# lan496/torch-m3gnet

Measured on AMD Instinct MI355X. Metric: atom-steps/sec (energy+forces) on 10k-atom PBC batch, 1/2/4/8 MI355X, higher is better.
Workload: dtype f32; 1 GPU; single 10000-atom fcc Cu PBC supercell per GPU (10x10x25 cells, a=3.61 A, jitter 0.025 A), r_cut 5 A / 3-body 4 A, default M3GNet (l_max=n_max=3, D=64, 3 blocks), energy+forces+stress; precision=fp32, atoms_per_gpu=10000, edges_per_gpu=420000, triplets_per_gpu=3060000

## Files before the change

torch-m3gnet_amd/csrc/m3g_api.hip:

```cpp
#include <climits>
#include <cmath>
#include <cstdarg>
#include <cstdio>
#include <cstdlib>
#include <cstring>
#include <utility>

#include "m3g_internal.h"

namespace m3g {

static thread_local char g_err[512] = "";
void set_error(const char* fmt, ...) {
  va_list ap;
  va_start(ap, fmt);
  vsnprintf(g_err, sizeof(g_err), fmt, ap);
  va_end(ap);
}

static void layout_mlp(MlpW& m, size_t& off) {
  auto take = [&](size_t n) { size_t r = off; off += (n + 63) / 64 * 64; return r; };
  m.w1a_t = take(kDP * 2 * kDP); m.w1b_t = take(kDP * 2 * kDP); m.w1c_t = take(kDP * 2 * kDP);
  m.b1 = take(2 * kDP);
  m.w2d_t = take(kDP * kDP); m.w2g_t = take(kDP * kDP);
// ... 304 lines not shown
  *value = *value == 0 ? 0 : *value == 3 ? 3 : *value == 2 ? 2 : 1;
  return M3G_OK;
}
struct OptionRow {
  const char* name;
  int Options::*member;
  int lo, hi;
  const char* error;
  int (*hook)(m3g_plan*, int32_t* value);
};
#define M3G_HOOK(...) [](m3g_plan* plan, int32_t* value) -> int { __VA_ARGS__; return M3G_OK; }
static const OptionRow kOptions[] = {
    {"edge_kernel", &Options::edge_kernel, 0, 2, "edge_kernel must be 0 (VALU baseline), 1 (MFMA) or 2 (any-size path)",
     M3G_HOOK(if (plan->generic && *value != 2) { set_error("this model size only runs on the any-size path (edge_kernel = 2)"); return M3G_ERR_UNSUPPORTED; })},
    {"precision", &Options::precision, 0, 2,
     "precision must be 0 (fp32: exact fp32 MFMA products), 1 (bf16x3 split products) or 2 (f16x3: scaled fp16 split products)", nullptr},
    {"save_p1", &Options::save_p1, 0, 1, nullptr, nullptr},
    {"save_p2", &Options::save_p2, 0, 1, nullptr, nullptr},
    {"rev_kernel", &Options::rev_kernel, 0, 1, "rev_kernel must be 0 (node-MLP + edge-MLP kernel pair) or 1 (fused)", nullptr},
    {"small_tiles", &Options::small_tiles, 0, INT_MAX, "small_tiles must be >= 0", M3G_HOOK(plan->opt.small_tiles_fwd = *value)},
    {"small_tiles_fwd", &Options::small_tiles_fwd, 0, INT_MAX, "small_tiles_fwd must be >= 0", nullptr},
    {"dp1_by_dst", &Options::dp1_by_dst, 0, 1, nullptr, nullptr},
    {"split_node_tiles", &Options::split_node_tiles, 0, INT_MAX, "split_node_tiles must be >= 0", nullptr},
    {"fuse_node_tb", &Options::fuse_node_tb, 0, 1, nullptr, nullptr},
    {"debug_node_tb_polls", &Options::debug_node_tb_polls, INT_MIN, INT_MAX, nullptr, nullptr},
    {"split_tail", &Options::split_tail, 0, 2, "split_tail must be 0 (never), 1 (a single left-over tile) or 2 (one or two)", nullptr},
    {"small_launches", &Options::small_launches, 0, 1, nullptr, nullptr},
    {"graph_replay", &Options::graph_replay, 0, 1, nullptr, M3G_HOOK(if (!*value) drop_graphs(plan))},
    {"overlap", &Options::overlap, 0, 1, nullptr, nullptr},
    {"threebody_moments", &Options::tb_moments, 0, 1, nullptr, nullptr},
    {"legendre_backward", &Options::legendre_ref, 0, 1, "legendre_backward: 0 (exact derivative) or 1 (the reference's backward)", nullptr},
    {"readout_f16", &Options::readout_f16, 0, 1, nullptr, nullptr},
    {"stress_mode", &Options::stress_mode, 0, 1, "stress_mode must be 0 (reference: sum pos (x) F / V) or 1 (pair virial)", nullptr},
    {"debug_force_move", nullptr, INT_MIN, INT_MAX, nullptr, M3G_HOOK(plan->debug_force_move = *value != 0; plan->committed = false)},
    {"stamps", &Options::stamp_target, INT_MIN, INT_MAX, nullptr, hook_stamps},
};
#undef M3G_HOOK

extern "C" int m3g_plan_set_option(m3g_plan* plan, const char* name, int32_t value) {
  if (!plan || !name) { set_error("m3g_plan_set_option: null argument"); return M3G_ERR_VALUE; }
  for (const OptionRow& row : kOptions) {
    if (strcmp(name, row.name) != 0) continue;
    if (value < row.lo || value > row.hi) {
      if (row.error) { set_error("%s", row.error); return M3G_ERR_VALUE; }
      value = 1;
    }
// ... 81 lines not shown
    std::string ro = buf;
    const float* wd0 = plan->params.at(ro + ".dense.0.weight").data();
    const float* wg0 = plan->params.at(ro + ".gate.0.weight").data();
    const float* wd2 = plan->params.at(ro + ".dense.2.weight").data();
    const float* wg2 = plan->params.at(ro + ".gate.2.weight").data();
    put_t(blob, r.w1d_t, kDP, wd0, D, D, 0, D); put_t(blob, r.w1g_t, kDP, wg0, D, D, 0, D);
    put_t(blob, r.w2d_t, kDP, wd2, D, D, 0, D); put_t(blob, r.w2g_t, kDP, wg2, D, D, 0, D);
    put_n(blob, r.w1d, kDP, wd0, D, D, 0, D); put_n(blob, r.w1g, kDP, wg0, D, D, 0, D);
    put_n(blob, r.w2d, kDP, wd2, D, D, 0, D); put_n(blob, r.w2g, kDP, wg2, D, D, 0, D);
    for (int o = 0; o < D; ++o) {
      blob[r.b1d + o] = plan->params.at(ro + ".dense.0.bias")[o];
      blob[r.b1g + o] = plan->params.at(ro + ".gate.0.bias")[o];
      blob[r.b2d + o] = plan->params.at(ro + ".dense.2.bias")[o];
      blob[r.b2g + o] = plan->params.at(ro + ".gate.2.bias")[o];
      blob[r.w3d + o] = plan->params.at(ro + ".dense.4.weight")[o];
      blob[r.w3g + o] = plan->params.at(ro + ".gate.4.weight")[o];
    }
    blob[r.b3] = plan->params.at(ro + ".dense.4.bias")[0];
    blob[r.b3 + 1] = plan->params.at(ro + ".gate.4.bias")[0];
  }
  if (!plan->d_weights) M3G_HIP_CHECK(hipMalloc((void**)&plan->d_weights, wl.total * sizeof(float)));
  M3G_HIP_CHECK(hipMemcpy(plan->d_weights, blob.data(), wl.total * sizeof(float), hipMemcpyHostToDevice));
  { int rc = pack_mfma_images(plan); if (rc) return rc; }
  plan->committed = true;
  return M3G_OK;
}

static StepPath plan_step_path(const m3g_plan* plan, int64_t N, int64_t E, int64_t T, int64_t S, int topo_hints, bool forces, bool stresses, bool profile) {
  const m3g_config& cfg = plan->cfg;
  return resolve_step_path(plan->opt, ModelDims{cfg.l_max, cfg.n_max, cfg.l_max * cfg.n_max, cfg.num_blocks}, N, E, T, S, topo_hints, forces, stresses, profile);
}

extern "C" int m3g_workspace_bytes(const m3g_plan* plan, int64_t N, int64_t E, int64_t T, int64_t S, size_t* bytes) {
  if (!plan || !bytes || N < 0 || E < 0 || T < 0 || S < 0) { set_error("m3g_workspace_bytes: bad argument"); return M3G_ERR_VALUE; }
  const StepPath p = plan_step_path(plan, N, E, T, S, 0, true, true, false);
  *bytes = p.pipeline == kPipeAnySize ? generic_workspace_bytes(plan, N, E, T, S) : work_carve(plan->cfg.num_blocks, p, N, E, S, nullptr).total_bytes;
  return M3G_OK;
}

static bool ensure_side_stream(const m3g_plan* plan) {
  if (plan->side_stream) return true;
  if (hipStreamCreateWithFlags(&plan->side_stream, hipStreamNonBlocking) != hipSuccess) { plan->side_stream = nullptr; return false; }
  if (hipEventCreateWithFlags(&plan->ev_fork, hipEventDisableTiming) != hipSuccess ||
      hipEventCreateWithFlags(&plan->ev_join, hipEventDisableTiming) != hipSuccess)
    return false;
  return true;
// ... 19 lines not shown
  const float* W;
  hipStream_t s;
  RunMode mode;
  Topo t;
  Work w;
  float *ea, *st;
  int enqueue_forward() const, enqueue_optional_outputs() const, enqueue_reverse() const;
};

static int check_call(const m3g_plan* plan, const m3g_io* io) {
  if (!plan || !io) { set_error("m3g_energy_forces: null argument"); return M3G_ERR_VALUE; }
  if (!plan->committed) { set_error("m3g_energy_forces: plan parameters not committed"); return M3G_ERR_STATE; }
  int dev = -1;
  M3G_HIP_CHECK(hipGetDevice(&dev));
  if (dev == plan->device) return M3G_OK;
  set_error("m3g_energy_forces: the plan was committed on device %d but the current device is %d (commit again on this device)", plan->device, dev);
  return M3G_ERR_STATE;
}

int Step::enqueue_forward() const {
  const bool want_f = io->forces != nullptr;
  {
    M3G_STAGE(ST_GEOM);
    if (p.geom_with_node_pre) launch_geometry_node_pre(plan, c, t, w, io->pos, io->lattice, io->edge_cell_shift, io->atom_types, W + wl.emb, s);
    else launch_geometry(c, t, io->pos, io->lattice, io->edge_cell_shift, w, s);
  }
  {
    M3G_STAGE(ST_EMBED);
    if (mfma) {
      if (c.B == 0) launch_embed_nodes_only(c, W, wl, t, io->atom_types, w, s);
      if (!p.fused_rev || c.B == 0) launch_embed_edges_soa(c, W + wl.adj_t, w.h, w.e_blk[0], t.E, s);
    } else {
      launch_embed(c, W, wl, t, io->atom_types, w, s);
    }
  }
  for (int b = 0; b < c.B; ++b) {
    {
      M3G_STAGE(ST_NODE_PRE);
      if (mfma && b == 0 && p.geom_with_node_pre) {  }
      else if (mfma) launch_node_pre_mfma(plan, p.node_split, c, t, w, b, b > 0 ? w.x[b - 1] : nullptr, w.x[b], w.v[b], w.TAb[b], w.TBb[b],
                                          b == 0 ? io->atom_types : nullptr, W + wl.emb, s);
      else launch_node_pre(c, W, wl.blk[b], t, w, nullptr, w.x[b], w.v[b], w.TA, w.TB, s);
    }
    { M3G_STAGE(ST_THREEBODY); launch_threebody(p, c, t, w, w.v[b], w.m[b], s); }
    M3G_STAGE(ST_EDGE_FWD);
    if (mfma) {
      if (p.fwd_split) launch_edge_fwd_split(plan, p, c, t, w, b, s);
      else launch_edge_block_mfma(plan, p, c, t, w, b, s);
      (void)ST_NODE_SUM;
    } else {
      launch_edge_block(c, W, wl.blk[b], t, w, b, w.x[b], w.x[b + 1], s);
    }
  }
  M3G_STAGE(ST_READOUT);
  if (mfma) launch_readout_mfma(plan, p, c, wl, t, io->atom_types, c.B > 0 ? w.x[c.B - 1] : nullptr, w.x[c.B], w, ea, st, io->total_energy, want_f, s);
  else launch_readout(c, W, wl, t, io->atom_types, nullptr, w.x[c.B], w, ea, st, io->total_energy, want_f, s);
  return M3G_OK;
}

int Step::enqueue_optional_outputs() const {
  M3G_STAGE(ST_OUTPUTS);
  if (io->node_features) launch_copy_strided(w.x[c.B], kDP, io->node_features, c.D, c.D, t.N, s);
  if (io->edge_attr) {
    if (mfma) launch_soa_to_rows(w.e_blk[c.B], io->edge_attr, c.D, c.D, t.E, s);
    else launch_copy_strided(w.e, kDP, io->edge_attr, c.D, c.D, t.E, s);
  }
  if (io->edge_distances && t.E > 0) M3G_HIP_CHECK(hipMemcpyAsync(io->edge_distances, w.d, sizeof(float) * t.E, hipMemcpyDeviceToDevice, s));
  if (io->edge_weights) launch_copy_strided(w.h, kRP, io->edge_weights, c.R, c.R, t.E, s);
  if (io->triplet_angles) launch_triplet_angles(t, io->triplet_edge_index, w.u, io->triplet_angles, s);
  if (io->mid_edge_features)
    for (int b = 0; b < c.B; ++b)
// ... 215 lines not shown
```

torch-m3gnet_amd/csrc/m3g_edge_mfma.hip:

```cpp
#include "m3g_edge_common.h"

namespace m3g {

__device__ __forceinline__ void save_store(float* ptr, const f32x4& val) { __builtin_nontemporal_store(val, (f32x4*)ptr); }
template <bool KEEP_P1, int PREC, int SAVE = 0>
__device__ __forceinline__ void mlp_preacts(const float* lds, int w1c, int w2d, int w2g, int b2, const f32x4 (&x)[4], f32x4 (&p1)[8],
                                            f32x4 (&p2)[8], int lane, float* p1_out = nullptr, float* p2_out = nullptr, float w_inv = 1.f) {
  chain_p<PREC, 8, 2>(lds + w1c, x, p1, lane, w_inv);
  if constexpr (SAVE == 1) static_for<8>([&]<int ob>() { *(f32x4*)(p1_out + ob * 256) = p1[ob]; });
  bias_step<4, 0>(lds + b2, p2, lane);
  bias_step<4, 4>(lds + b2 + 4 * 64, p2, lane);
  if constexpr (!KEEP_P1 && SAVE == 2) {
    static_for<8>([&]<int ob>() {
      f32x4 ds;
      static_for<2>([&]<int k>() {
        f32x2 act, der;
        silu_pair(f32x2{p1[ob][2 * k], p1[ob][2 * k + 1]}, act, der);
        p1[ob][2 * k] = act[0]; p1[ob][2 * k + 1] = act[1];
        ds[2 * k] = der[0]; ds[2 * k + 1] = der[1];
      });
      save_store(p1_out + ob * 256, ds);
    });
    chain_p<PREC, 4, 2, 0, 0>(lds + w2d, p1, p2, lane, w_inv);
    chain_p<PREC, 4, 2, 4, 4>(lds + w2g, p1, p2, lane, w_inv);
// ... 17 lines not shown
      static_for<8>([&]<int ob>() { static_for<4>([&]<int r>() { p1[ob][r] = fsilu(p1[ob][r]); }); });
    }
    chain_p<PREC, 4, 2, 0, 0>(lds + w2d, p1, p2, lane, w_inv);
    chain_p<PREC, 4, 2, 4, 4>(lds + w2g, p1, p2, lane, w_inv);
  }
}

template <bool ST, int S0, int PREC, int SAVE>
__device__ __forceinline__ void mlp_forward_mfma(const float* lds, const MfmaMlpFwd& L, int mlp, const FwdArgs& a, int64_t ci,
                                                 int64_t cj, float hb, const f32x4 (&x)[4], f32x4 (&out)[4], int lane,
                                                 Stamps<ST>& st, float* p1_out, float* p2_out) {
  f32x4 p1[8], p2[8];
  gather_tables(a.TA, a.TB, mlp, ci, cj, lane >> 4, p1);
  st.template mark<S0>();
  mlp_preacts<false, PREC, SAVE>(lds, L.w1c, L.w2d, L.w2g, L.b2, x, p1, p2, lane, p1_out, p2_out, a.w_inv);
  st.template mark<S0 + 1>();
  static_for<4>([&]<int ob>() {
    out[ob] = mfma16(lds[L.wl + ob * 64 + lane], hb, zero4());
    mul_gated<PREC == kPrecF16x3 || PREC == kPrecF32>(out[ob], p2[ob], p2[4 + ob]);
  });
  st.template mark<S0 + 3>();
}

template <int TBS, bool ST = false, bool FIRST = false, int PREC = kPrecBf16x3, int SAVE = 0>
__global__ void __launch_bounds__(64 * fwd_waves<PREC>()) k_edge_block_mfma(FwdArgs a, MfmaFwdLayout L) {
  __shared__ __attribute__((aligned(16))) float lds[kFwdLdsFloats + 4];
  int* q_head = reinterpret_cast<int*>(lds + kFwdLdsFloats);
  load_image(lds, a.img, kFwdLdsFloats, q_head);
  const int lane = threadIdx.x & 63, qd = lane >> 4;
  TileQueue queue(a.tiles, q_head);
  Stamps<ST> st;
  int ticket = queue.fetch(lane);
  if (ticket >= queue.count) return;
  int ci_i, cj_i;
  load_ends(a.src, a.dst, queue.base + ticket, a.E, lane, ci_i, cj_i);
  int arow_i = load_arow(a.act_id, queue.base + ticket, a.E, lane);
  for (;;) {
    const int64_t tile = queue.base + ticket;
    ticket = queue.fetch(lane);
    const bool has_next = ticket < queue.count;
    int nci = 0, ncj = 0, narow = -1;
    if (has_next) {
      load_ends(a.src, a.dst, queue.base + ticket, a.E, lane, nci, ncj);
      narow = load_arow(a.act_id, queue.base + ticket, a.E, lane);
    }
    int lv = lane;
    asm volatile("" : "+v"(lv));
// ... 9 lines not shown
    if (!FIRST) static_for<4>([&]<int blk>() { x[blk] = load_tile4(e_tile + blk * 256); });
    const int arow = arow_i;
    const TbIn<PREC, TBS> tbin = tb_load<PREC, TBS>(a.m, arow, qv, a.w_inv);
    const float hb = a.h[ec * kRP + qv];
    if (FIRST) {
      static_for<4>([&]<int blk>() {
        x[blk] = mfma16(lds[L.adj + blk * 64 + lv], hb, zero4());
        static_for<4>([&]<int r>() { x[blk][r] = fsilu(x[blk][r]); });
      });
    }
    st.template mark<0>();
    {
      f32x4 p[8];
      tb_preact_p<PREC, TBS>(lds + L.tb, tbin, p, lv);
      static_for<4>([&]<int blk>() { add_gated<PREC == kPrecF16x3 || PREC == kPrecF32>(x[blk], p[blk], p[4 + blk]); });
    }
    st.template mark<1>();
    f32x4 out[4];
    float* p1_tile = SAVE >= 1 ? a.p1_out + tile * (2 * kP1TileFloats) + lane * 4 : nullptr;
    float* p2_tile = SAVE >= 2 ? a.p2_out + tile * (2 * kP1TileFloats) + lane * 4 : nullptr;
    mlp_forward_mfma<ST, 2, PREC, SAVE>(lds, L.mlp[0], 0, a, ci, cj, hb, x, out, lv, st, p1_tile, p2_tile);
    static_for<4>([&]<int blk>() {
      x[blk] += out[blk];
      *(f32x4*)(e_otile + blk * 256) = x[blk];
    });
    st.template mark<6>();
    mlp_forward_mfma<ST, 7, PREC, SAVE>(lds, L.mlp[1], 1, a, ci, cj, hb, x, out, lv, st, SAVE >= 1 ? p1_tile + kP1TileFloats : nullptr,
                                        SAVE >= 2 ? p2_tile + kP1TileFloats : nullptr);
    {
      if (edge >= a.E) static_for<4>([&]<int blk>() { out[blk] = zero4(); });
      const SegMasks sk = seg_masks((int)ci, lane);
      seg_scan(out, sk);
      seg_store(out, sk, a.seg_head, a.seg_first, tile, ci, qd, 0);
    }
    st.template mark<11>();
    if (!has_next) break;
    ci_i = nci;
    cj_i = ncj;
    arow_i = narow;
  }
  st.template store<false>(a.stamps, lane);
}

template <bool ST, int PREC, bool SAVED>
__device__ __forceinline__ void mlp_reverse_mfma(const float* lds, const MfmaMlpRev& L, int mlp, const RevArgs& a, int64_t edge, int64_t tile,
                                                 int64_t ci, int64_t cj, const f32x4& hv, const f32x4 (&x)[4],
                                                 const f32x4 (&d_upd)[4], f32x4 (&contrib)[4], f32x4& dhv, int lane,
// ... 428 lines not shown
  d0 += __shfl_xor(d0, 32); d1 += __shfl_xor(d1, 32); d2 += __shfl_xor(d2, 32); d3 += __shfl_xor(d3, 32);
  if (qd == 0 && edge < E) *(f32x4*)(dh + edge * kRP) = f32x4{d0, d1, d2, d3};
}

void launch_rows_to_soa(const float* rows, float* soa, int64_t E, hipStream_t s) {
  int64_t tiles = tiles_for(E);
  if (tiles > 0)
    hipLaunchKernelGGL(k_rows_to_soa, dim3((unsigned)((tiles * kTileFloats + 255) / 256)), dim3(256), 0, s, E, tiles, rows, soa);
}
void launch_soa_to_rows(const float* soa, float* rows, int row_stride, int width, int64_t E, hipStream_t s) {
  if (E > 0) hipLaunchKernelGGL(k_soa_to_rows, dim3((unsigned)((E * kDP + 255) / 256)), dim3(256), 0, s, E, width, row_stride, soa, rows);
}
void launch_embed_edges_soa(const Consts& c, const float* adj_t, const float* h, float* soa, int64_t E, hipStream_t s) {
  int64_t tiles = tiles_for(E);
  if (tiles > 0)
    hipLaunchKernelGGL(k_embed_edges_soa, dim3((unsigned)((tiles * kTileFloats + 255) / 256)), dim3(256), 0, s, c.R, E, tiles, adj_t, h, soa);
}
void launch_embed_edges_reverse_soa(const float* adj, const float* h, const float* de_soa, float* dh, int64_t E, hipStream_t s) {
  int64_t tiles = tiles_for(E);
  if (tiles > 0)
    hipLaunchKernelGGL(k_embed_edges_reverse_soa, dim3((unsigned)((tiles * 64 + 255) / 256)), dim3(256), 0, s, E, tiles, adj, h, de_soa, dh);
}

void launch_edge_block_mfma(const m3g_plan* plan, const StepPath& p, const Consts& c, const Topo& t, const Work& w, int b, hipStream_t s) {
  const int64_t tiles = tiles_for(t.E);
  const MfmaFwdLayout L = mfma_fwd_layout();
  const int prec = plan->opt.precision;
  if (tiles > 0) {
    FwdArgs a = fwd_args(t, w, b, plan->d_mfma_fwd[prec] + (size_t)b * L.total);
    a.stamps = plan->d_stamps;
    if (p.saved_acts >= 1) a.p1_out = w.p1_blk[b];
    if (p.saved_acts == 2) a.p2_out = w.p2_blk[b];
    if (prec == kPrecF16x3) a.w_inv = plan->w_scale_inv;
    dim3 grid(grid_for_tiles(tiles));
    const bool first = b == 0 && p.fused_rev;
    const int save = p.fwd_save;
#define M3G_FWD_LAUNCH(ST_, FIRST_, PREC_, SAVE_) hipLaunchKernelGGL((k_edge_block_mfma<TBS, ST_, FIRST_, PREC_, SAVE_>), grid, dim3(64 * fwd_waves<PREC_>()), 0, s, a, L)
#define M3G_FWD_BY_MODE(ST_, FIRST_)                                                               \
  if (prec == kPrecBf16x3) { M3G_FWD_LAUNCH(ST_, FIRST_, kPrecBf16x3, 0); }                        \
  else if (prec == kPrecF16x3) { M3G_FWD_LAUNCH(ST_, FIRST_, kPrecF16x3, 0); }                     \
  else if (save == 2) { M3G_FWD_LAUNCH(ST_, FIRST_, kPrecF32, 2); }                                \
  else if (save == 1) { M3G_FWD_LAUNCH(ST_, FIRST_, kPrecF32, 1); }                                \
  else { M3G_FWD_LAUNCH(ST_, FIRST_, kPrecF32, 0); }
    if (plan->d_stamps && plan->opt.stamp_target == 1 && tb_steps_for(c.C) == 3) {
      constexpr int TBS = 3;
      if (first) { M3G_FWD_BY_MODE(true, true); } else { M3G_FWD_BY_MODE(true, false); }
    } else if (first) {
      M3G_TBS_SWITCH(c.C, M3G_FWD_BY_MODE(false, true));
    } else {
      M3G_TBS_SWITCH(c.C, M3G_FWD_BY_MODE(false, false));
    }
#undef M3G_FWD_BY_MODE
#undef M3G_FWD_LAUNCH
  }
}

void launch_edge_rev_node_mlp(const m3g_plan* plan, const StepPath& p, const Consts& c, const Topo& t, const Work& w, int b, const float* dx_new,
                              hipStream_t s) {
  (void)c;
  const int64_t tiles = tiles_for(t.E);
  if (tiles == 0) return;
  const MfmaRevLayout L = mfma_rev_layout();
  const int prec = plan->opt.precision;
// ... 59 lines not shown
```

torch-m3gnet_amd/csrc/m3g_internal.h:

```cpp
#pragma once
#include <hip/hip_runtime.h>

#include <cmath>
#include <cstddef>
#include <cstdint>
#include <map>
#include <string>
#include <vector>

#include "../../include/m3gnet_hip.h"
#include "m3g_step_path.h"

namespace m3g {

constexpr int kDP = 64;
constexpr int kLCap = 4;
constexpr int kRCap = 4;
constexpr int kCP = 16;
constexpr int kRP = 4;

void set_error(const char* fmt, ...);
#define M3G_HIP_CHECK(expr)                                                               \
  do {                                                                                    \
    hipError_t _e = (expr);                                                               \
// ... 95 lines not shown
  MfmaMlpFused mlp[2];
  int adj;
  int adjp;
  int total;
};
struct MfmaMlpRevF32 {
  int w2d, w2g;
  int w1cT;
  int b2;
  int wl;
  int wld;
};
struct MfmaRevF32Layout {
  int tb;
  int tbT;
  MfmaMlpRevF32 mlp[2];
  int adj;
  int adjp;
  int total;
};
MfmaRevF32Layout mfma_rev_f32_layout();
constexpr int kNodeRowBlocks = 33;
constexpr int kNodeImgFloats = kNodeRowBlocks * 16 * 64 + kNodeRowBlocks * 16;
struct ReadoutImg {
  static constexpr int w1 = 0;
  static constexpr int w2d = w1 + 8 * 2 * 512;
  static constexpr int w2g = w2d + 4 * 2 * 512;
  static constexpr int w2dT = w2g + 4 * 2 * 512;
  static constexpr int w2gT = w2dT + 4 * 2 * 512;
  static constexpr int w1T = w2gT + 4 * 2 * 512;
  static constexpr int b1 = w1T + 4 * 4 * 512;
  static constexpr int b2 = b1 + 128;
  static constexpr int w3 = b2 + 128;
  static constexpr int b3 = w3 + 128;
  static constexpr int total = b3 + 4;
};
MfmaFwdLayout mfma_fwd_layout();
MfmaRevLayout mfma_rev_layout();
MfmaRevFusedLayout mfma_rev_fused_layout();

}

struct m3g_plan {
  m3g_config cfg;
  m3g::Consts consts;
  m3g::WeightLayout wl;
  std::map<std::string, std::vector<float>> params;
  std::map<std::string, std::vector<float>> cvals;
  float* d_weights = nullptr;
  float* d_mfma_fwd[m3g::kNumPrec] = {nullptr, nullptr, nullptr};
  float* d_mfma_rev[m3g::kNumPrec] = {nullptr, nullptr, nullptr};
  float* d_mfma_revf = nullptr;
  float* d_mfma_revf_h = nullptr;
  float* d_mfma_revf32 = nullptr;
  float* d_node_img[m3g::kNumPrec] = {nullptr, nullptr, nullptr};
  m3g::Options opt;
  float w_scale_inv = 1.f;
  int device = -1;
  bool generic = false;
  float* d_generic = nullptr;
  std::map<std::string, size_t> generic_off;
  float* d_readout_img = nullptr;
  float* d_readout_img_h = nullptr;
  float ro_w_scale_inv = 1.f;
  unsigned long long* d_stamps = nullptr;
  bool committed = false;
  bool debug_force_move = false;
  mutable hipStream_t side_stream = nullptr;
  mutable hipEvent_t ev_fork = nullptr, ev_join = nullptr;
  struct GraphEntry { std::vector<unsigned char> key; hipGraph_t graph = nullptr; hipGraphExec_t exec = nullptr; };
  mutable std::vector<GraphEntry> graphs;
  bool profile = false;
  mutable std::vector<hipEvent_t> ev_pool;
  mutable std::vector<int> ev_stage;
  mutable size_t ev_used = 0;
};

namespace m3g {
// ... 139 lines not shown
                             bool dr_done = false);
void launch_stress(const Consts& c, const Topo& t, const float* pos, const float* lattice, const float* forces,
                   float* stresses, hipStream_t s, const float* ea = nullptr, float* scaled_total = nullptr, float* total = nullptr);
void launch_stress_pair(const Topo& t, const Work& w, const float* lattice, float* stresses, hipStream_t s);
void launch_force_gather(float length_scale, const Topo& t, const float* dr, float* forces, float* stresses, hipStream_t s);
size_t generic_workspace_bytes(const m3g_plan* plan, int64_t N, int64_t E, int64_t T, int64_t S);
int generic_commit(m3g_plan* plan);
void generic_free(m3g_plan* plan);
int generic_energy_forces(const m3g_plan* plan, const m3g_io* io, void* workspace, size_t workspace_bytes, hipStream_t s);
void launch_triplet_angles(const Topo& t, const int64_t* tei, const float* u, float* out, hipStream_t s);
void launch_distance_only(float length_scale, const Topo& t, const float* pos, const float* lattice,
                          const int32_t* shift, float* u, float* d, hipStream_t s);
void launch_edge_featurizer(const Consts& c, int64_t E, const float* d, float* out, int out_stride, hipStream_t s);
void launch_embed(const Consts& c, const float* W, const WeightLayout& wl, const Topo& t, const int64_t* types,
                  const Work& w, hipStream_t s);
void launch_embed_reverse(const Consts& c, const float* W, const WeightLayout& wl, const Topo& t, const Work& w,
                          hipStream_t s);
void launch_node_pre(const Consts& c, const float* W, const BlockW& bw, const Topo& t, const Work& w, const float* x_prev, float* x,
                     float* v, float* TA, float* TB, hipStream_t s);
void launch_node_pre_mfma(const m3g_plan* plan, bool split, const Consts& c, const Topo& t, const Work& w, int b, const float* x_prev, float* x,
                          float* v, float* TA, float* TB, const int64_t* types, const float* emb, hipStream_t s);
void launch_geometry_node_pre(const m3g_plan* plan, const Consts& c, const Topo& t, const Work& w, const float* pos, const float* lattice,
                              const int32_t* shift, const int64_t* types, const float* emb, hipStream_t s);
void launch_energy_sums(const Consts& c, const Topo& t, const float* scaled_atomic, float* scaled_total, float* total, hipStream_t s);
void launch_readout_mfma(const m3g_plan* plan, const StepPath& p, const Consts& c, const WeightLayout& wl, const Topo& t, const int64_t* types,
                         const float* x_prev, float* x, const Work& w, float* scaled_atomic, float* scaled_total, float* total,
                         bool want_grad, hipStream_t s);
void launch_node_reverse(const Consts& c, const float* W, const BlockW& bw, const Topo& t, const Work& w,
                         const float* v, const float* dx_new, float* dx_out, bool row_sums_in_seg, int dp1_packed, bool with_v_term,
                         hipStream_t s, bool small = false);
void launch_node_reverse_v_term(const Consts& c, const float* W, const BlockW& bw, const Topo& t, const Work& w, const float* v,
                                float* dx_out, hipStream_t s);
void launch_readout(const Consts& c, const float* W, const WeightLayout& wl, const Topo& t, const int64_t* types,
                    const float* x_prev, float* x, const Work& w, float* scaled_atomic, float* scaled_total, float* total,
                    bool want_grad, hipStream_t s);
void launch_gather_rows(const float* table, int64_t n, int width, int table_stride, int table_rows, bool transposed,
                        const int64_t* idx, float* out, hipStream_t s);
void launch_copy_expand_rows(const int32_t* row_id, const float* in, int in_stride, float* out, int out_stride, int width, int64_t n,
                             hipStream_t s);
void launch_copy_strided(const float* in, int in_stride, float* out, int out_stride, int width, int64_t rows,
                         hipStream_t s);
void launch_threebody(const StepPath& p, const Consts& c, const Topo& t, const Work& w, const float* v, float* m, hipStream_t s);
void launch_threebody_reverse(const StepPath& p, const Consts& c, const Topo& t, const Work& w, const float* v, bool first, hipStream_t s,
                              bool ref_legendre = false);
void launch_threebody_reverse_final(const Consts& c, const Topo& t, const Work& w, const float* v, bool first, const float* dh, int dh_parts,
                                    hipStream_t s, int topo_hints);
bool launch_node_tb_reverse(const Consts& c, const float* W, const BlockW& bw, const Topo& t, const Work& w, const float* v, bool first,
                            const float* dx_new, float* dx_out, int dp1_packed, int block, hipStream_t s, int topo_hints, int debug_polls = 0);
int pack_mfma_images(m3g_plan* plan);
void free_mfma_images(m3g_plan* plan);
void launch_edge_block_mfma(const m3g_plan* plan, const StepPath& p, const Consts& c, const Topo& t, const Work& w, int b, hipStream_t s);
void launch_edge_rev_node_mlp(const m3g_plan* plan, const StepPath& p, const Consts& c, const Topo& t, const Work& w, int b, const float* dx_new,
                              hipStream_t s);
void launch_edge_rev_edge_mlp(const m3g_plan* plan, const StepPath& p, const Consts& c, const Topo& t, const Work& w, int b, const float* dx_new,
                              bool de_is_zero, hipStream_t s);
void launch_edge_rev_fused(const m3g_plan* plan, const Consts& c, const Topo& t, const Work& w, int b, const float* dx_new,
                           bool de_is_zero, hipStream_t s);
void launch_edge_rev_f32(const m3g_plan* plan, const StepPath& p, const Consts& c, const Topo& t, const Work& w, int b, const float* dx_new,
                         bool de_is_zero, hipStream_t s);
void launch_edge_fwd_split(const m3g_plan* plan, const StepPath& p, const Consts& c, const Topo& t, const Work& w, int b, hipStream_t s);
void launch_edge_rev_split(const m3g_plan* plan, const StepPath& p, const Consts& c, const Topo& t, const Work& w, int b, const float* dx_new, bool de_is_zero,
                           hipStream_t s);
void launch_embed_edges_soa(const Consts& c, const float* adj_t, const float* h, float* soa, int64_t E, hipStream_t s);
void launch_embed_edges_reverse_soa(const float* adj, const float* h, const float* de_soa, float* dh_slice, int64_t E, hipStream_t s);
void launch_embed_nodes_only(const Consts& c, const float* W, const WeightLayout& wl, const Topo& t, const int64_t* types,
                             const Work& w, hipStream_t s);
void launch_rows_to_soa(const float* rows, float* soa, int64_t E, hipStream_t s);
void launch_soa_to_rows(const float* soa, float* rows, int row_stride, int width, int64_t E, hipStream_t s);
void launch_edge_block(const Consts& c, const float* W, const BlockW& bw, const Topo& t, const Work& w, int b,
                       const float* x_old, float* x_new, hipStream_t s);
void launch_edge_block_reverse(const Consts& c, const float* W, const BlockW& bw, const Topo& t, const Work& w, int b,
                               const float* dx_new, hipStream_t s);

}
// ... 1 lines not shown
```

torch-m3gnet_amd/csrc/m3g_node_mfma.hip:

```cpp
#include "m3g_edge_common.h"
#include "m3g_struct_sum.h"
#include "m3g_geometry_body.h"

namespace m3g {


constexpr int kNodeXPitch = 68;
__device__ __forceinline__ void add_message_sums(f32x4 (&xr)[4], int64_t atom, int q, const float* __restrict__ seg_head,
                                                 const float* __restrict__ seg_first, const int32_t* __restrict__ row_ptr) {
  const int r0 = row_ptr[atom], r1 = row_ptr[atom + 1];
  if (r1 > r0) {
    if (r0 & 15) static_for<4>([&]<int j>() { xr[j] += *(const f32x4*)(seg_first + atom * (4 * kDP) + 16 * q + 4 * j); });
    for (int t = (r0 + 15) >> 4; t <= (r1 - 1) >> 4; ++t)
      static_for<4>([&]<int j>() { xr[j] += *(const f32x4*)(seg_head + (int64_t)t * (4 * kDP) + 16 * q + 4 * j); });
  }
}
__device__ __forceinline__ void store_x_row(float* __restrict__ x, int64_t atom, int q, const f32x4 (&xr)[4]) {
  static_for<4>([&]<int j>() { *(f32x4*)(x + atom * kDP + 16 * q + 4 * j) = xr[j]; });
}
__device__ __forceinline__ void x_rows_to_blocks(float* xs, int m, int q, const f32x4 (&xr)[4], f32x4 (&xb)[4]) {
  static_for<4>([&]<int j>() { *(f32x4*)(xs + m * kNodeXPitch + 16 * q + 4 * j) = xr[j]; });
  static_for<4>([&]<int blk>() { xb[blk] = *(const f32x4*)(xs + m * kNodeXPitch + blk * 16 + 4 * q); });
}
__device__ __forceinline__ void store_node_block(int ob, const f32x4& acc, int64_t atom, int q, int C, float* __restrict__ TA, float* __restrict__ TB,
// ... 129 lines not shown
  f32x4 xb[4];
  x_rows_to_blocks(xs, m, q, xr, xb);
  static_for<4>([&]<int blk>() {
    static_for<4>([&]<int r>() {
      const float b = xb[blk][r];
      static_for<3>([&]<int jj>() { acc[jj] = mfma16(a[jj][blk * 4 + r], b, acc[jj]); });
    });
  });
  if (!live) return;
  static_for<3>([&]<int jj>() {
    const int j = w + 4 * jj;
    if (j >= 11) return;
    store_node_block(11 * g + j, acc[jj], atom, q, C, TA, TB, v);
  });
}

__global__ void __launch_bounds__(256) k_node_pre_split(NodePreArgs a) { node_pre_split_body(a, blockIdx.x); }
template <int L, int R>
__global__ void __launch_bounds__(256) k_geometry_node_pre(Consts c, GeomArgs ga, int n_geo, NodePreArgs na) {
  if ((int)blockIdx.x < n_geo) geometry_body<true, L, R>(c, ga, blockIdx.x);
  else node_pre_split_body(na, (int64_t)blockIdx.x - n_geo);
}

struct ReadoutSums {
  const int32_t *struct_ptr, *flags, *batch;
  float* total;
  int32_t* counter;
};
template <int PREC>
__global__ void __launch_bounds__(256) k_readout_mfma(Consts c, int64_t N, const float* __restrict__ img, float w_inv, const float* __restrict__ elemental,
                                                      const int64_t* __restrict__ types, const float* __restrict__ x_prev,
                                                      const float* __restrict__ seg_head, const float* __restrict__ seg_first,
                                                      const int32_t* __restrict__ row_ptr, float* __restrict__ x,
                                                      float* scaled_atomic, float* __restrict__ dx,
                                                      float* __restrict__ scaled_total, int64_t S, ReadoutSums rs) {
  __shared__ __attribute__((aligned(16))) float lds[ReadoutImg::total + 4 * 16 * kNodeXPitch];
  if (blockIdx.x == 0) for (int64_t i = threadIdx.x; i < S; i += blockDim.x) scaled_total[i] = 0.f;
  {
    constexpr int kVec = ReadoutImg::total / 4, kBatch = 16;
    for (int base = 0; base < kVec; base += 256 * kBatch) {
      f32x4 t[kBatch];
      static_for<kBatch>([&]<int j>() {
        const int i = base + j * 256 + (int)threadIdx.x;
        t[j] = i < kVec ? *(const f32x4*)(img + 4 * i) : zero4();
      });
      static_for<kBatch>([&]<int j>() {
// ... 240 lines not shown
    const NodePreArgs a{c.C, t.N, plan->d_node_img[kPrecF32] + (size_t)b * kNodeImgFloats, x_prev, w.seg_head, w.seg_first, t.row_ptr, x, v, TA, TB,
                        types, emb, c.num_types};
    hipLaunchKernelGGL(k_node_pre_split, dim3((unsigned)(3 * tiles)), dim3(256), 0, s, a);
    return;
  }
  const int wgs = 3 * (int)std::min<int64_t>((tiles + 3) / 4, 256);
  M3G_PREC_SWITCH(prec,
                  hipLaunchKernelGGL((k_node_pre_mfma<PREC>), dim3(wgs), dim3(256), 0, s, c.C, t.N,
                                     plan->d_node_img[prec] + (size_t)b * kNodeImgFloats, x_prev, w.seg_head, w.seg_first,
                                     t.row_ptr, x, v, TA, TB, types, emb, c.num_types,
                                     prec == kPrecF16x3 ? plan->w_scale_inv : 1.f));
}

void launch_geometry_node_pre(const m3g_plan* plan, const Consts& c, const Topo& t, const Work& w, const float* pos, const float* lattice,
                              const int32_t* shift, const int64_t* types, const float* emb, hipStream_t s) {
  const int64_t tiles = (t.N + 15) / 16;
  const int n_geo = (int)((t.E + 255) / 256);
  const GeomArgs ga = geometry_args(t, pos, lattice, shift, w);
  const NodePreArgs na{c.C, t.N, plan->d_node_img[kPrecF32], nullptr, w.seg_head, w.seg_first, t.row_ptr, w.x[0], w.v[0], w.TAb[0], w.TBb[0], types, emb,
                       c.num_types};
  M3G_DISPATCH_LR(c.L, c.R, hipLaunchKernelGGL((k_geometry_node_pre<L, R>), dim3((unsigned)(n_geo + 3 * tiles)), dim3(256), 0, s, c, ga, n_geo, na));
}

}
```

torch-m3gnet_amd/csrc/m3g_pack_mfma.hip:

```cpp
#include <cmath>
#include <cstring>

#include "m3g_dual_chain.h"
#include "m3g_dual_f32.h"
#include "m3g_internal.h"

namespace m3g {

MfmaFwdLayout mfma_fwd_layout() {
  MfmaFwdLayout L{};
  int off = 0;
  auto take = [&](int n) { int r = off; off += n; return r; };
  L.tb = take(8 * kTbSteps * 64);
  for (int m = 0; m < 2; ++m) {
    L.mlp[m].w1c = take(8 * 4 * 4 * 64);
    L.mlp[m].w2d = take(4 * 4 * 4 * 64);
    L.mlp[m].w2g = take(4 * 4 * 4 * 64);
    L.mlp[m].b2 = take(2 * 4 * 64);
    L.mlp[m].wl = take(4 * 1 * 64);
  }
  L.adj = take(4 * 64);
  L.total = off;
  return L;
}
// ... 113 lines not shown
static void direct_image(float* img, int OB, int S, F get) {
  for (int ob = 0; ob < OB; ++ob)
    for (int s = 0; s < S; ++s)
      for (int lane = 0; lane < 64; ++lane) img[(ob * S + s) * 64 + lane] = get(ob * 16 + (lane & 15), 4 * s + (lane >> 4));
}

template <class F>
static void f32_chain_image(float* img, int OB, int S, F get) {
  for (int ob = 0; ob < OB; ++ob)
    for (int s = 0; s < S; ++s)
      for (int lane = 0; lane < 64; ++lane)
        img[(ob * S + s) * 64 + lane] = get(ob * 16 + (lane & 15), (s >> 2) * 16 + 4 * (lane >> 4) + (s & 3));
}

template <class F>
static void chain_image_p(int prec, float wscale, float* img, int OB, int KS, F get) {
  if (prec == kPrecBf16x3) chain_image(img, OB, KS, get);
  else if (prec == kPrecF16x3) chain_image_h(img, OB, KS, wscale, get);
  else f32_chain_image(img, OB, 8 * KS, get);
}

void free_mfma_images(m3g_plan* plan) {
  auto drop = [](float*& p) { if (p) { (void)hipFree(p); p = nullptr; } };
  for (int prec = 0; prec < kNumPrec; ++prec) { drop(plan->d_mfma_fwd[prec]); drop(plan->d_mfma_rev[prec]); drop(plan->d_node_img[prec]); }
  drop(plan->d_mfma_revf);
  drop(plan->d_mfma_revf_h);
  drop(plan->d_mfma_revf32);
  drop(plan->d_readout_img);
  drop(plan->d_readout_img_h);
}

static int upload(float*& dst, const std::vector<float>& host) {
  if (!dst) M3G_HIP_CHECK(hipMalloc((void**)&dst, host.size() * sizeof(float)));
  M3G_HIP_CHECK(hipMemcpy(dst, host.data(), host.size() * sizeof(float), hipMemcpyHostToDevice));
  return M3G_OK;
}

int pack_mfma_images(m3g_plan* plan) {
  const m3g_config& cfg = plan->cfg;
  const int D = cfg.embedding_dim, R = cfg.n_max, C = cfg.l_max * cfg.n_max, B = cfg.num_blocks;
  const MfmaFwdLayout F = mfma_fwd_layout();
  const MfmaRevLayout Rv = mfma_rev_layout();
  const MfmaRevFusedLayout Rf = mfma_rev_fused_layout();
  const MfmaRevF32Layout R32 = mfma_rev_f32_layout();
  std::vector<float> revf((size_t)std::max(B, 1) * Rf.total, 0.f), revf32((size_t)std::max(B, 1) * R32.total, 0.f);
  std::vector<float> revfh((size_t)std::max(B, 1) * Rf.total, 0.f);
  float wscale = 1.f;
// ... 206 lines not shown
```

torch-m3gnet_amd/csrc/m3g_step_path.h:

```cpp
#pragma once
#include <cstdint>

#include "../../include/m3gnet_hip.h"

namespace m3g {

constexpr int kMaxBlocks = 8;
constexpr int kPrecF32 = 0;
constexpr int kPrecBf16x3 = 1;
constexpr int kPrecF16x3 = 2;
constexpr int kNumPrec = 3;

constexpr int kSyncWords = 16;
constexpr int kSyncForceTail = 0, kSyncReadout = 1, kSyncNodeRev = 2;
constexpr int64_t kForceTailMaxStructs = 8;
constexpr int64_t kFusedSumsMaxAtoms = 1024;
constexpr int64_t kNodeTbFusedMaxAtoms = 128;

constexpr int32_t topo_hints_word(int32_t bad, int32_t rows, int32_t atoms) {
  return (bad == 0 && rows > 0) ? (M3G_TOPO_TB_COMPLETE | ((rows & 0xff) << 8) | ((atoms & 0xff) << 16)) : 0;
}
constexpr int topo_hints_rows(int hints) { return (hints >> 8) & 0xff; }
constexpr int topo_hints_atoms(int hints) { return (hints >> 16) & 0xff; }

struct Options {
  int precision = kPrecF32;
  int save_p1 = 1;
  int save_p2 = 1;
  int small_tiles_fwd = 3072;
  int small_tiles = 1536;
  int dp1_by_dst = 0;
  int split_node_tiles = 128;
  int fuse_node_tb = 1;
  int debug_node_tb_polls = 0;
  int split_tail = 1;
  int small_launches = 1;
  int rev_kernel = 1;
  int readout_f16 = 0;
  int legendre_ref = 0;
  int tb_moments = 1;
  int stress_mode = 0;
  int edge_kernel = 1;
  int stamp_target = 0;
  int overlap = 0;
  int graph_replay = 0;
};
static_assert(sizeof(Options) == 20 * sizeof(int), "Options: twenty ints, no padding (its bytes are compared as a key)");

enum { kDp1F32 = 0, kDp1Packed = 1, kDp1Fixed = 2, kDp1F32ByDst = 3  };

enum Pipeline { kPipeValu = 0, kPipeMfma = 1, kPipeAnySize = 2 };
enum RevEdge { kRevValu = 0, kRevPair, kRevFused, kRevF32, kRevSplit };
enum Readout { kReadoutValu = 0, kReadoutSplit, kReadoutF32, kReadoutF16 };
enum RevTail {
  kTailSeparate = 0,
  kTailOverlap,
  kTailNodeTb,
  kTailFinalTb,
};
enum StressKernel { kStressNone = 0, kStressInGather , kStressPair, kStressRef };

struct ModelDims { int L, R, C, B; };

struct StepPath {
  int pipeline = kPipeMfma;
  bool fused_rev = false;
  int saved_acts = 0;
  int fwd_save = 0;
  int dp1 = kDp1F32;
  bool dp1_by_dst = false;
  int tb_hints = 0;
  bool moments = false;
  bool long_lists = false;
  bool geom_with_node_pre = false;
  bool node_split = false;
  bool fwd_split = false;
  int rev_edge = kRevValu;
  int split_tail = 0;
  int readout = kReadoutValu;
  bool readout_sums = false;
  bool energy_deferred = false;
  int tail[kMaxBlocks] = {};
  bool node_rev_small = false;
  bool gather_virial = false;
  int stress = kStressNone;
};

inline StepPath resolve_step_path(const Options& o, const ModelDims& m, int64_t N, int64_t E, int64_t T, int64_t S, int topo_hints,
                                  bool want_forces, bool want_stresses, bool profile) {
  StepPath p;
  p.pipeline = o.edge_kernel;
  if (o.edge_kernel == 2) return p;
  const bool mfma = o.edge_kernel == 1, f32 = o.precision == kPrecF32, stamps = o.stamp_target != 0;
  const bool saves_p1 = mfma && f32 && o.save_p1 != 0;
  const bool saves_p2 = saves_p1 && o.rev_kernel == 1 && o.save_p2 != 0;
  p.saved_acts = saves_p2 ? 2 : saves_p1 ? 1 : 0;
  p.fwd_save = want_forces ? p.saved_acts : 0;
  p.fused_rev = mfma && o.rev_kernel == 1 && (!f32 || saves_p1);
  p.dp1_by_dst = o.dp1_by_dst && p.fused_rev && f32;
  p.dp1 = !p.fused_rev ? kDp1F32 : p.dp1_by_dst ? kDp1F32ByDst : o.precision == kPrecBf16x3 ? kDp1Packed : o.precision == kPrecF16x3 ? kDp1Fixed : kDp1F32;

  p.tb_hints = o.tb_moments && !o.legendre_ref ? topo_hints : 0;
  p.moments = (p.tb_hints & M3G_TOPO_TB_COMPLETE) && m.L >= 1 && m.L <= 3 && m.R >= 1 && m.R <= 4 && topo_hints_rows(p.tb_hints) > 0 &&
              topo_hints_atoms(p.tb_hints) > 0;
  p.long_lists = T > 24 * E;
  const bool tb_mom = p.moments && E != 0 && T != 0;

  const int64_t etiles = (E + 15) / 16, ntiles = (N + 15) / 16;
  const bool small_nodes = o.small_launches && ntiles <= o.split_node_tiles;
  const bool few = N <= kFusedSumsMaxAtoms && S > 0 && S <= kForceTailMaxStructs;
  if (mfma) {
    p.node_split = f32 && small_nodes;
    p.geom_with_node_pre = !profile && p.node_split && m.B != 0 && E != 0 && N != 0;
    p.fwd_split = etiles > 0 && etiles <= o.small_tiles_fwd && f32 && p.fwd_save != 1 && !stamps;
    p.rev_edge = !p.fused_rev ? kRevPair : !f32 ? kRevFused : (etiles > 0 && etiles <= o.small_tiles && saves_p2 && !stamps) ? kRevSplit : kRevF32;
    p.split_tail = o.split_tail;
    const bool f16_readout = o.precision == kPrecF16x3 && o.readout_f16;
    p.readout = f16_readout ? kReadoutF16 : small_nodes ? kReadoutSplit : kReadoutF32;
    p.readout_sums = o.small_launches && N > 0 && few;
    p.energy_deferred = o.small_launches && want_forces && want_stresses && o.stress_mode == 0 && !profile && !p.readout_sums && N > 0;
  }
  if (!want_forces) return p;
  for (int b = 0; b < m.B && b < kMaxBlocks; ++b) {
    if (b > 0 && p.fused_rev && o.overlap && !profile) p.tail[b] = kTailOverlap;
    else if (b > 0 && p.fused_rev && o.fuse_node_tb && !profile && N <= kNodeTbFusedMaxAtoms && N != 0 && tb_mom && kSyncNodeRev + b < kSyncWords)
      p.tail[b] = kTailNodeTb;
    else if (b == 0 && p.fused_rev && o.small_launches && !profile && tb_mom) p.tail[b] = kTailFinalTb;
  }
  p.node_rev_small = o.small_launches && N <= kFusedSumsMaxAtoms;
  p.gather_virial = mfma && o.small_launches && o.stress_mode == 0 && want_stresses && N > 0 && few;
  p.stress = !want_stresses ? kStressNone : p.gather_virial ? kStressInGather : o.stress_mode == 1 ? kStressPair : kStressRef;
  return p;
}

}
```

Before: 4.169 million atom-steps/s.

## Precompute per-species block-0 node tables and skip unread last-block edge store

At commit time, runs the block-0 node-pre MLP once per atom species and stores the results (x, v, TA, TB rows) in a per-precision table. Each step then fills block-0 node inputs by gathering from that table, fused into the geometry launch when edges exist, instead of running the node-pre MFMA kernel. Separately, the last edge-forward block no longer writes updated edge features when nothing reads them, which removes a large store. This is valid because block-0 node features depend only on atom type, and it adds table memory plus a new option that is on by default.

```diff
diff --git a/torch-m3gnet_amd/csrc/m3g_api.hip b/torch-m3gnet_amd/csrc/m3g_api.hip
--- a/torch-m3gnet_amd/csrc/m3g_api.hip
+++ b/torch-m3gnet_amd/csrc/m3g_api.hip
@@ -350,6 +350,7 @@
     {"small_tiles_fwd", &Options::small_tiles_fwd, 0, INT_MAX, "small_tiles_fwd must be >= 0", nullptr},
     {"dp1_by_dst", &Options::dp1_by_dst, 0, 1, nullptr, nullptr},
     {"split_node_tiles", &Options::split_node_tiles, 0, INT_MAX, "split_node_tiles must be >= 0", nullptr},
+    {"species_tables", &Options::species_tables, 0, 1, nullptr, nullptr},
     {"fuse_node_tb", &Options::fuse_node_tb, 0, 1, nullptr, nullptr},
     {"debug_node_tb_polls", &Options::debug_node_tb_polls, INT_MIN, INT_MAX, nullptr, nullptr},
     {"split_tail", &Options::split_tail, 0, 2, "split_tail must be 0 (never), 1 (a single left-over tile) or 2 (one or two)", nullptr},
@@ -477,6 +478,7 @@
   if (!plan->d_weights) M3G_HIP_CHECK(hipMalloc((void**)&plan->d_weights, wl.total * sizeof(float)));
   M3G_HIP_CHECK(hipMemcpy(plan->d_weights, blob.data(), wl.total * sizeof(float), hipMemcpyHostToDevice));
   { int rc = pack_mfma_images(plan); if (rc) return rc; }
+  { int rc = build_species_tables(plan); if (rc) return rc; }
   plan->committed = true;
   return M3G_OK;
 }
@@ -542,7 +544,8 @@
   const bool want_f = io->forces != nullptr;
   {
     M3G_STAGE(ST_GEOM);
-    if (p.geom_with_node_pre) launch_geometry_node_pre(plan, c, t, w, io->pos, io->lattice, io->edge_cell_shift, io->atom_types, W + wl.emb, s);
+    if (p.block0 == kBlock0ExpandBesideGeom) launch_geometry_species(plan, c, t, w, io->pos, io->lattice, io->edge_cell_shift, io->atom_types, s);
+    else if (p.block0 == kBlock0Kernel && p.geom_with_node_pre) launch_geometry_node_pre(plan, c, t, w, io->pos, io->lattice, io->edge_cell_shift, io->atom_types, W + wl.emb, s);
     else launch_geometry(c, t, io->pos, io->lattice, io->edge_cell_shift, w, s);
   }
   {
@@ -557,7 +560,9 @@
   for (int b = 0; b < c.B; ++b) {
     {
       M3G_STAGE(ST_NODE_PRE);
-      if (mfma && b == 0 && p.geom_with_node_pre) {  }
+      if (mfma && b == 0 && p.block0 == kBlock0ExpandBesideGeom) {  }
+      else if (mfma && b == 0 && p.block0 == kBlock0ExpandAlone) launch_species_expand(plan, c, t, w, io->atom_types, s);
+      else if (mfma && b == 0 && p.geom_with_node_pre) {  }
       else if (mfma) launch_node_pre_mfma(plan, p.node_split, c, t, w, b, b > 0 ? w.x[b - 1] : nullptr, w.x[b], w.v[b], w.TAb[b], w.TBb[b],
                                           b == 0 ? io->atom_types : nullptr, W + wl.emb, s);
       else launch_node_pre(c, W, wl.blk[b], t, w, nullptr, w.x[b], w.v[b], w.TA, w.TB, s);
@@ -566,7 +571,7 @@
     M3G_STAGE(ST_EDGE_FWD);
     if (mfma) {
       if (p.fwd_split) launch_edge_fwd_split(plan, p, c, t, w, b, s);
-      else launch_edge_block_mfma(plan, p, c, t, w, b, s);
+      else launch_edge_block_mfma(plan, p, c, t, w, b, s, b + 1 < c.B || io->edge_attr != nullptr);
       (void)ST_NODE_SUM;
     } else {
       launch_edge_block(c, W, wl.blk[b], t, w, b, w.x[b], w.x[b + 1], s);
diff --git a/torch-m3gnet_amd/csrc/m3g_edge_mfma.hip b/torch-m3gnet_amd/csrc/m3g_edge_mfma.hip
--- a/torch-m3gnet_amd/csrc/m3g_edge_mfma.hip
+++ b/torch-m3gnet_amd/csrc/m3g_edge_mfma.hip
@@ -63,7 +63,7 @@
   st.template mark<S0 + 3>();
 }
 
-template <int TBS, bool ST = false, bool FIRST = false, int PREC = kPrecBf16x3, int SAVE = 0>
+template <int TBS, bool ST = false, bool FIRST = false, int PREC = kPrecBf16x3, int SAVE = 0, bool STORE_E = true>
 __global__ void __launch_bounds__(64 * fwd_waves<PREC>()) k_edge_block_mfma(FwdArgs a, MfmaFwdLayout L) {
   __shared__ __attribute__((aligned(16))) float lds[kFwdLdsFloats + 4];
   int* q_head = reinterpret_cast<int*>(lds + kFwdLdsFloats);
@@ -119,7 +119,7 @@
     mlp_forward_mfma<ST, 2, PREC, SAVE>(lds, L.mlp[0], 0, a, ci, cj, hb, x, out, lv, st, p1_tile, p2_tile);
     static_for<4>([&]<int blk>() {
       x[blk] += out[blk];
-      *(f32x4*)(e_otile + blk * 256) = x[blk];
+      if constexpr (STORE_E) *(f32x4*)(e_otile + blk * 256) = x[blk];
     });
     st.template mark<6>();
     mlp_forward_mfma<ST, 7, PREC, SAVE>(lds, L.mlp[1], 1, a, ci, cj, hb, x, out, lv, st, SAVE >= 1 ? p1_tile + kP1TileFloats : nullptr,
@@ -594,7 +594,8 @@
     hipLaunchKernelGGL(k_embed_edges_reverse_soa, dim3((unsigned)((tiles * 64 + 255) / 256)), dim3(256), 0, s, E, tiles, adj, h, de_soa, dh);
 }
 
-void launch_edge_block_mfma(const m3g_plan* plan, const StepPath& p, const Consts& c, const Topo& t, const Work& w, int b, hipStream_t s) {
+void launch_edge_block_mfma(const m3g_plan* plan, const StepPath& p, const Consts& c, const Topo& t, const Work& w, int b, hipStream_t s,
+                            bool e_out_read) {
   const int64_t tiles = tiles_for(t.E);
   const MfmaFwdLayout L = mfma_fwd_layout();
   const int prec = plan->opt.precision;
@@ -611,6 +612,7 @@
 #define M3G_FWD_BY_MODE(ST_, FIRST_)                                                               \
   if (prec == kPrecBf16x3) { M3G_FWD_LAUNCH(ST_, FIRST_, kPrecBf16x3, 0); }                        \
   else if (prec == kPrecF16x3) { M3G_FWD_LAUNCH(ST_, FIRST_, kPrecF16x3, 0); }                     \
+  else if (save == 2 && !ST_ && !e_out_read) { hipLaunchKernelGGL((k_edge_block_mfma<TBS, false, FIRST_, kPrecF32, 2, false>), grid, dim3(64 * fwd_waves<kPrecF32>()), 0, s, a, L); } \
   else if (save == 2) { M3G_FWD_LAUNCH(ST_, FIRST_, kPrecF32, 2); }                                \
   else if (save == 1) { M3G_FWD_LAUNCH(ST_, FIRST_, kPrecF32, 1); }                                \
   else { M3G_FWD_LAUNCH(ST_, FIRST_, kPrecF32, 0); }
diff --git a/torch-m3gnet_amd/csrc/m3g_internal.h b/torch-m3gnet_amd/csrc/m3g_internal.h
--- a/torch-m3gnet_amd/csrc/m3g_internal.h
+++ b/torch-m3gnet_amd/csrc/m3g_internal.h
@@ -141,6 +141,10 @@
 MfmaRevF32Layout mfma_rev_f32_layout();
 constexpr int kNodeRowBlocks = 33;
 constexpr int kNodeImgFloats = kNodeRowBlocks * 16 * 64 + kNodeRowBlocks * 16;
+constexpr int kSpeciesRowFloats = kDP + kCP + 2 * 4 * kDP;
+constexpr size_t species_tab_v(int num_types) { return (size_t)num_types * kDP; }
+constexpr size_t species_tab_ta(int num_types) { return (size_t)num_types * (kDP + kCP); }
+constexpr size_t species_tab_tb(int num_types) { return (size_t)num_types * (kDP + kCP + 4 * kDP); }
 struct ReadoutImg {
   static constexpr int w1 = 0;
   static constexpr int w2d = w1 + 8 * 2 * 512;
@@ -173,6 +177,7 @@
   float* d_mfma_revf_h = nullptr;
   float* d_mfma_revf32 = nullptr;
   float* d_node_img[m3g::kNumPrec] = {nullptr, nullptr, nullptr};
+  float* d_species_tab[m3g::kNumPrec] = {nullptr, nullptr, nullptr};
   m3g::Options opt;
   float w_scale_inv = 1.f;
   int device = -1;
@@ -358,6 +363,10 @@
                           float* v, float* TA, float* TB, const int64_t* types, const float* emb, hipStream_t s);
 void launch_geometry_node_pre(const m3g_plan* plan, const Consts& c, const Topo& t, const Work& w, const float* pos, const float* lattice,
                               const int32_t* shift, const int64_t* types, const float* emb, hipStream_t s);
+void launch_species_expand(const m3g_plan* plan, const Consts& c, const Topo& t, const Work& w, const int64_t* types, hipStream_t s);
+void launch_geometry_species(const m3g_plan* plan, const Consts& c, const Topo& t, const Work& w, const float* pos, const float* lattice,
+                             const int32_t* shift, const int64_t* types, hipStream_t s);
+int build_species_tables(m3g_plan* plan);
 void launch_energy_sums(const Consts& c, const Topo& t, const float* scaled_atomic, float* scaled_total, float* total, hipStream_t s);
 void launch_readout_mfma(const m3g_plan* plan, const StepPath& p, const Consts& c, const WeightLayout& wl, const Topo& t, const int64_t* types,
                          const float* x_prev, float* x, const Work& w, float* scaled_atomic, float* scaled_total, float* total,
@@ -385,7 +394,8 @@
                             const float* dx_new, float* dx_out, int dp1_packed, int block, hipStream_t s, int topo_hints, int debug_polls = 0);
 int pack_mfma_images(m3g_plan* plan);
 void free_mfma_images(m3g_plan* plan);
-void launch_edge_block_mfma(const m3g_plan* plan, const StepPath& p, const Consts& c, const Topo& t, const Work& w, int b, hipStream_t s);
+void launch_edge_block_mfma(const m3g_plan* plan, const StepPath& p, const Consts& c, const Topo& t, const Work& w, int b, hipStream_t s,
+                            bool e_out_read = true);
 void launch_edge_rev_node_mlp(const m3g_plan* plan, const StepPath& p, const Consts& c, const Topo& t, const Work& w, int b, const float* dx_new,
                               hipStream_t s);
 void launch_edge_rev_edge_mlp(const m3g_plan* plan, const StepPath& p, const Consts& c, const Topo& t, const Work& w, int b, const float* dx_new,
diff --git a/torch-m3gnet_amd/csrc/m3g_node_mfma.hip b/torch-m3gnet_amd/csrc/m3g_node_mfma.hip
--- a/torch-m3gnet_amd/csrc/m3g_node_mfma.hip
+++ b/torch-m3gnet_amd/csrc/m3g_node_mfma.hip
@@ -175,6 +175,59 @@
   else node_pre_split_body(na, (int64_t)blockIdx.x - n_geo);
 }
 
+struct SpeciesArgs {
+  int64_t N;
+  const int64_t* types;
+  int num_types;
+  const float* tab;
+  float *x, *v, *TA, *TB;
+};
+constexpr int kSpeciesRowVecs = kSpeciesRowFloats / 4, kSpeciesVecsPerThread = 4;
+__device__ __forceinline__ void species_expand_body(const SpeciesArgs& a, int64_t vblock) {
+  const int64_t total = a.N * kSpeciesRowVecs;
+  const int64_t first = vblock * (256 * kSpeciesVecsPerThread) + threadIdx.x;
+  const float* __restrict__ tab = a.tab;
+  const int64_t* __restrict__ types = a.types;
+  const int nt = a.num_types;
+  f32x4 t[kSpeciesVecsPerThread];
+  float* dst[kSpeciesVecsPerThread];
+  static_for<kSpeciesVecsPerThread>([&]<int j>() {
+    const int64_t i = first + j * 256;
+    dst[j] = nullptr;
+    if (i >= total) return;
+    const int64_t atom = i / kSpeciesRowVecs;
+    const int piece = (int)(i - atom * kSpeciesRowVecs);
+    bool bad;
+    const int64_t ty = species_index(types[atom], nt, bad);
+    const float* src;
+    if (piece < 16) {
+      src = tab + ty * kDP + 4 * piece;
+      dst[j] = a.x + atom * kDP + 4 * piece;
+    } else if (piece < 20) {
+      src = tab + species_tab_v(nt) + ty * kCP + 4 * (piece - 16);
+      dst[j] = a.v + atom * kCP + 4 * (piece - 16);
+    } else if (piece < 84) {
+      src = tab + species_tab_ta(nt) + ty * (4 * kDP) + 4 * (piece - 20);
+      dst[j] = a.TA + atom * (4 * kDP) + 4 * (piece - 20);
+    } else {
+      src = tab + species_tab_tb(nt) + ty * (4 * kDP) + 4 * (piece - 84);
+      dst[j] = a.TB + atom * (4 * kDP) + 4 * (piece - 84);
+    }
+    t[j] = *(const f32x4*)src;
+  });
+  static_for<kSpeciesVecsPerThread>([&]<int j>() {
+    if (dst[j]) *(f32x4*)dst[j] = t[j];
+  });
+}
+static_assert(kSpeciesRowVecs == 16 + 4 + 64 + 64, "species_expand_body: the pieces of a row");
+
+__global__ void __launch_bounds__(256) k_species_expand(SpeciesArgs a) { species_expand_body(a, blockIdx.x); }
+template <int L, int R>
+__global__ void __launch_bounds__(256) k_geometry_species(Consts c, GeomArgs ga, int n_geo, SpeciesArgs sa) {
+  if ((int)blockIdx.x < n_geo) geometry_body<true, L, R>(c, ga, blockIdx.x);
+  else species_expand_body(sa, (int64_t)blockIdx.x - n_geo);
+}
+
 struct ReadoutSums {
   const int32_t *struct_ptr, *flags, *batch;
   float* total;
@@ -461,4 +514,49 @@
   M3G_DISPATCH_LR(c.L, c.R, hipLaunchKernelGGL((k_geometry_node_pre<L, R>), dim3((unsigned)(n_geo + 3 * tiles)), dim3(256), 0, s, c, ga, n_geo, na));
 }
 
-}
+static SpeciesArgs species_args(const m3g_plan* plan, const Consts& c, const Topo& t, const Work& w, const int64_t* types) {
+  return SpeciesArgs{t.N, types, c.num_types, plan->d_species_tab[plan->opt.precision], w.x[0], w.v[0], w.TAb[0], w.TBb[0]};
+}
+static unsigned species_expand_blocks(int64_t N) {
+  constexpr int64_t per = 256 * kSpeciesVecsPerThread;
+  return (unsigned)((N * kSpeciesRowVecs + per - 1) / per);
+}
+void launch_species_expand(const m3g_plan* plan, const Consts& c, const Topo& t, const Work& w, const int64_t* types, hipStream_t s) {
+  hipLaunchKernelGGL(k_species_expand, dim3(species_expand_blocks(t.N)), dim3(256), 0, s, species_args(plan, c, t, w, types));
+}
+void launch_geometry_species(const m3g_plan* plan, const Consts& c, const Topo& t, const Work& w, const float* pos, const float* lattice,
+                             const int32_t* shift, const int64_t* types, hipStream_t s) {
+  const int n_geo = (int)((t.E + 255) / 256);
+  const GeomArgs ga = geometry_args(t, pos, lattice, shift, w);
+  const SpeciesArgs sa = species_args(plan, c, t, w, types);
+  M3G_DISPATCH_LR(c.L, c.R, hipLaunchKernelGGL((k_geometry_species<L, R>), dim3((unsigned)n_geo + species_expand_blocks(t.N)), dim3(256), 0, s, c, ga, n_geo, sa));
+}
+
+int build_species_tables(m3g_plan* plan) {
+  const int nt = plan->cfg.num_types;
+  if (plan->cfg.num_blocks == 0) return M3G_OK;
+  std::vector<int64_t> iota(nt);
+  for (int i = 0; i < nt; ++i) iota[i] = i;
+  int64_t* d_types = nullptr;
+  M3G_HIP_CHECK(hipMalloc((void**)&d_types, sizeof(int64_t) * nt));
+  hipError_t e = hipMemcpy(d_types, iota.data(), sizeof(int64_t) * nt, hipMemcpyHostToDevice);
+  const int64_t tiles = (nt + 15) / 16;
+  const int wgs = 3 * (int)std::min<int64_t>((tiles + 3) / 4, 256);
+  for (int prec = 0; prec < kNumPrec && e == hipSuccess; ++prec) {
+    float*& tab = plan->d_species_tab[prec];
+    if (!tab) e = hipMalloc((void**)&tab, sizeof(float) * (size_t)nt * kSpeciesRowFloats);
+    if (e != hipSuccess) break;
+    M3G_PREC_SWITCH(prec,
+                    hipLaunchKernelGGL((k_node_pre_mfma<PREC>), dim3(wgs), dim3(256), 0, nullptr, plan->consts.C, (int64_t)nt, plan->d_node_img[prec],
+                                       nullptr, nullptr, nullptr, nullptr, tab, tab + species_tab_v(nt), tab + species_tab_ta(nt),
+                                       tab + species_tab_tb(nt), d_types, plan->d_weights + plan->wl.emb, nt,
+                                       prec == kPrecF16x3 ? plan->w_scale_inv : 1.f));
+    e = hipGetLastError();
+  }
+  if (e == hipSuccess) e = hipDeviceSynchronize();
+  (void)hipFree(d_types);
+  M3G_HIP_CHECK(e);
+  return M3G_OK;
+}
+
+}
diff --git a/torch-m3gnet_amd/csrc/m3g_pack_mfma.hip b/torch-m3gnet_amd/csrc/m3g_pack_mfma.hip
--- a/torch-m3gnet_amd/csrc/m3g_pack_mfma.hip
+++ b/torch-m3gnet_amd/csrc/m3g_pack_mfma.hip
@@ -159,7 +159,7 @@
 
 void free_mfma_images(m3g_plan* plan) {
   auto drop = [](float*& p) { if (p) { (void)hipFree(p); p = nullptr; } };
-  for (int prec = 0; prec < kNumPrec; ++prec) { drop(plan->d_mfma_fwd[prec]); drop(plan->d_mfma_rev[prec]); drop(plan->d_node_img[prec]); }
+  for (int prec = 0; prec < kNumPrec; ++prec) { drop(plan->d_mfma_fwd[prec]); drop(plan->d_mfma_rev[prec]); drop(plan->d_node_img[prec]); drop(plan->d_species_tab[prec]); }
   drop(plan->d_mfma_revf);
   drop(plan->d_mfma_revf_h);
   drop(plan->d_mfma_revf32);
diff --git a/torch-m3gnet_amd/csrc/m3g_step_path.h b/torch-m3gnet_amd/csrc/m3g_step_path.h
--- a/torch-m3gnet_amd/csrc/m3g_step_path.h
+++ b/torch-m3gnet_amd/csrc/m3g_step_path.h
@@ -31,6 +31,7 @@
   int small_tiles = 1536;
   int dp1_by_dst = 0;
   int split_node_tiles = 128;
+  int species_tables = 1;
   int fuse_node_tb = 1;
   int debug_node_tb_polls = 0;
   int split_tail = 1;
@@ -45,7 +46,7 @@
   int overlap = 0;
   int graph_replay = 0;
 };
-static_assert(sizeof(Options) == 20 * sizeof(int), "Options: twenty ints, no padding (its bytes are compared as a key)");
+static_assert(sizeof(Options) == 21 * sizeof(int), "Options: twenty-one ints, no padding (its bytes are compared as a key)");
 
 enum { kDp1F32 = 0, kDp1Packed = 1, kDp1Fixed = 2, kDp1F32ByDst = 3  };
 
@@ -57,6 +58,11 @@
   kTailOverlap,
   kTailNodeTb,
   kTailFinalTb,
+};
+enum Block0Tables {
+  kBlock0Kernel = 0,
+  kBlock0ExpandBesideGeom,
+  kBlock0ExpandAlone,
 };
 enum StressKernel { kStressNone = 0, kStressInGather , kStressPair, kStressRef };
 
@@ -73,6 +79,7 @@
   bool moments = false;
   bool long_lists = false;
   bool geom_with_node_pre = false;
+  int block0 = kBlock0Kernel;
   bool node_split = false;
   bool fwd_split = false;
   int rev_edge = kRevValu;
@@ -112,6 +119,7 @@
   if (mfma) {
     p.node_split = f32 && small_nodes;
     p.geom_with_node_pre = !profile && p.node_split && m.B != 0 && E != 0 && N != 0;
+    if (o.species_tables && m.B != 0 && N != 0) p.block0 = !profile && E != 0 ? kBlock0ExpandBesideGeom : kBlock0ExpandAlone;
     p.fwd_split = etiles > 0 && etiles <= o.small_tiles_fwd && f32 && p.fwd_save != 1 && !stamps;
     p.rev_edge = !p.fused_rev ? kRevPair : !f32 ? kRevFused : (etiles > 0 && etiles <= o.small_tiles && saves_p2 && !stamps) ? kRevSplit : kRevF32;
     p.split_tail = o.split_tail;
```

Result: faster. 4.239 million atom-steps/s, median of 6 (+1.7%).
